# bcgsc/ntJoin

Hardware: AMD Instinct MI355X
Metric: Gbp/s minimizer-sketch+graph-build (k=32,w=1000) (higher is better)
Workload: dtype u64

## Files before the change

ntjoin_amd/csrc/graph.hip:

```cpp
#include <algorithm>
#include <cstdlib>
#include <cstring>
#include <system_error>
#include <thread>

#include "join_verdict.h"
#include "graph_rank.h"
#include "mxg_internal.h"
#include "scan_kernels.h"

namespace mxg {

static constexpr uint64_t HT_EMPTY = 0xFFFFFFFFFFFFFFFFull;
static constexpr uint32_t NONE32 = 0xFFFFFFFFu;

struct Slot {
    unsigned long long key;
    uint32_t nseen, ndup;
};

__device__ __forceinline__ uint32_t ht_slot(Slot *tab, uint32_t mask, uint32_t cap, uint64_t key)
{
    if (key == HT_EMPTY) return cap;
    uint32_t s = (uint32_t)((key * 0x9E3779B97F4A7C15ull) >> 32) & mask;
// ... 65 lines not shown

__global__ __launch_bounds__(256) void k_flags(const AsmSet p, const Slot *__restrict__ tab, uint32_t *cnt, uint32_t *sup)
{
    const uint32_t a = asm_of_block(p, blockIdx.x);
    const uint32_t i = (blockIdx.x - p.bstart[a]) * 256u + threadIdx.x;
    bool sh = false;
    if (i < asm_n(p, a)) {
        const uint32_t bit = 1u << a, full = p.full;
        const Slot sl = tab[p.slot[a][i]];
        const uint32_t seen = ~sl.nseen & full, d = ~sl.ndup & full;
        const bool uniq = !(d & bit);
        const bool inall = seen == full;
        sh = inall && d == 0;
        p.flags[a][i] = (uint8_t)((uniq ? MXG_MX_UNIQUE : 0) | (sh ? MXG_MX_SHARED : 0) | (inall ? MXG_MX_INALL : 0));
    }
    const uint32_t c = (uint32_t)__syncthreads_count(sh ? 1 : 0);
    if (threadIdx.x == 0) count_publish(cnt + p.bstart[a], sup + sup_start(p, a), blockIdx.x - p.bstart[a], c);
}


__device__ __forceinline__ uint32_t pj_part(uint64_t key, uint32_t pmask)
{
    return (uint32_t)((key * 0x9E3779B97F4A7C15ull) >> 44) & pmask;
}

constexpr uint32_t PJ_REC_DUP = 0x80000000u;
__device__ __forceinline__ uint32_t pj_run_role(uint32_t i, uint32_t n, uint64_t key, bool live)
{
    const uint32_t lane = threadIdx.x & 63u;
    const uint64_t prev = __shfl_up(key, 1), next = __shfl_down(key, 1);
    const bool fol = live && lane > 0 && prev == key;
    const bool lead = live && !fol && lane < 63 && i + 1 < n && next == key;
    return (fol ? 1u : 0u) | (lead ? 2u : 0u);
}

constexpr uint32_t PJ_BT = 1024;
__global__ __launch_bounds__(PJ_BT) void k_pj_bucket(const AsmSet p, uint32_t nb, uint32_t pmask, uint32_t *M, uint4 *recs,
                                                   uint32_t *sup, uint32_t n_sup)
{
    extern __shared__ uint32_t pj_lds[];
    uint32_t *hist = pj_lds, *start = pj_lds + pmask + 1;
    __shared__ uint32_t sh[256];
    if (blockIdx.x == 0)
        for (uint32_t i = threadIdx.x; i < n_sup; i += PJ_BT) sup[i] = 0;
    constexpr uint32_t U = PJ_IPB / PJ_BT;
    constexpr uint32_t BPU = PJ_BT / 256;
    const uint32_t j = blockIdx.x, sub = threadIdx.x >> 8, t256 = threadIdx.x & 255u;
    const uint32_t blk0 = j * (PJ_IPB / 256), a0 = asm_of_block(p, blk0), a1 = asm_of_block(p, min(blk0 + PJ_IPB / 256, nb) - 1u);
    const bool one = a0 == a1;
    const uint64_t *hp0 = p.hash[a0];
    uint32_t *sp0 = p.slot[a0];
    const uint32_t n0 = asm_n(p, a0), ib0 = (blk0 - p.bstart[a0]) * 256u;
    uint64_t key[U];
    uint32_t live = 0, dupm = 0;
#pragma unroll
    for (uint32_t u = 0; u < U; ++u) {
        const uint32_t blk = blk0 + u * BPU + sub;
        key[u] = 0;
        if (blk >= nb) continue;
        const uint64_t *hp = hp0;
        uint32_t *sp = sp0;
        uint32_t i = ib0 + (u * BPU + sub) * 256u + t256, n = n0;
        if (!one) {
            const uint32_t a = asm_of_block(p, blk);
            hp = p.hash[a];
            sp = p.slot[a];
            i = (blk - p.bstart[a]) * 256u + t256;
            n = asm_n(p, a);
        }
        const bool lv = i < n;
        if (lv) {
            key[u] = hp[i];
            sp[i] = PJ_VERDICT_PREFILL;
        }
        const uint32_t role = pj_run_role(i, n, key[u], lv);
        const uint64_t fb = __ballot(role & 1u);
        if ((threadIdx.x & 63u) == 0) p.fol[(size_t)blk * 4u + ((threadIdx.x >> 6) & 3u)] = fb;
        if (lv && !(role & 1u)) live |= 1u << u;
        if (role & 2u) dupm |= 1u << u;
    }
    for (uint32_t b = threadIdx.x; b <= pmask; b += PJ_BT) hist[b] = 0;
    __syncthreads();
#pragma unroll
    for (uint32_t u = 0; u < U; ++u)
        if ((live >> u) & 1u) atomicAdd(&hist[pj_part(key[u], pmask)], 1u);
    __syncthreads();
    const uint32_t P = pmask + 1, per = P >= PJ_BT ? P / PJ_BT : 1u, b0 = threadIdx.x * per;
    uint32_t c = 0;
    if (b0 < P)
        for (uint32_t u = 0; u < per; ++u) c += hist[b0 + u];
    uint32_t run = block_exclusive<PJ_BT / 64>(c, sh);
    uint32_t *row = M + (size_t)j * (P + 1);
    if (b0 < P)
        for (uint32_t u = 0; u < per; ++u) {
            const uint32_t cb = hist[b0 + u];
            start[b0 + u] = run;
            row[b0 + u] = run;
            hist[b0 + u] = 0;
            run += cb;
        }
    if (threadIdx.x == 0) row[P] = sh[255];
    __syncthreads();
#pragma unroll
    for (uint32_t u = 0; u < U; ++u) {
        if (!((live >> u) & 1u)) continue;
        const uint32_t blk = blk0 + u * BPU + sub;
        uint32_t a = a0, i = ib0 + (u * BPU + sub) * 256u + t256;
        if (!one) {
            a = asm_of_block(p, blk);
            i = (blk - p.bstart[a]) * 256u + t256;
        }
        const uint32_t b = pj_part(key[u], pmask);
        const uint32_t pos = j * PJ_IPB + start[b] + atomicAdd(&hist[b], 1u);
        recs[pos] = make_uint4((uint32_t)key[u], (uint32_t)(key[u] >> 32), i, a | (((dupm >> u) & 1u) ? PJ_REC_DUP : 0u));
    }
}

__device__ __forceinline__ uint32_t pj_slot_from(unsigned long long *keys, uint64_t key, uint32_t s)
{
    if (key == HT_EMPTY) return PJ_T;
    for (uint32_t step = 0; step < PJ_T; ++step) {
        const unsigned long long cur = keys[s];
        if (cur == key) return s;
        if (cur == HT_EMPTY) {
            const unsigned long long old = atomicCAS(&keys[s], (unsigned long long)HT_EMPTY, (unsigned long long)key);
            if (old == HT_EMPTY || old == key) return s;
        }
        s = (s + 1u) & (PJ_T - 1u);
    }
    return PJ_T + 1u;
}
__device__ __forceinline__ uint32_t pj_slot(unsigned long long *keys, uint64_t key)
{
    return pj_slot_from(keys, key, (uint32_t)((key * 0x9E3779B97F4A7C15ull) >> 32) & (PJ_T - 1u));
}

struct PjRec3 {
    uint32_t x, y, z;
};
template <bool R12>
__device__ __forceinline__ uint4 pj_rec_load(const uint4 *recs, size_t r)
{
    if (!R12) return recs[r];
    const PjRec3 v = reinterpret_cast<const PjRec3 *>(recs)[r];
    return make_uint4(v.x, v.y, v.z, 0u);
}
template <bool R12>
__device__ __forceinline__ void pj_rec_store(uint4 *recs, size_t r, const uint4 v)
{
    if (!R12) recs[r] = v;
    else reinterpret_cast<PjRec3 *>(recs)[r] = PjRec3{v.x, v.y, v.z};
}

struct PjSub {
    uint32_t n_sub, s, off, cap;
};
struct PjSubCaps {
    uint32_t n_sub;
    uint32_t cap[MXG_MAX_ASSEMBLIES];
};
template <bool NARROW>
__global__ __launch_bounds__(256) void k_pj_join(uint4 *recs, const uint32_t *__restrict__ M, uint32_t P, uint32_t n_rows,
                                                 uint64_t *host_fail, uint32_t force_fail, const uint32_t *__restrict__ cursor,
                                                 uint32_t cap1, uint32_t rows2, const AsmSet p, const PjSubCaps caps, uint32_t prefill0)
{
    const uint32_t full = p.full;
    __shared__ unsigned long long keys[PJ_T + 1];
    __shared__ uint32_t seen[PJ_T + 1], dup[NARROW ? 1 : PJ_T + 1];
    __shared__ uint32_t item0[PJ_T + 1];
    __shared__ uint32_t seg_off[257], seg_rec[256], sh[256];
    __shared__ uint32_t failed;
    uint32_t b = blockIdx.x, rec_off = 0;
    if (cursor) {
        const uint32_t c = blockIdx.x / P;
        b = blockIdx.x % P;
        n_rows = caps.n_sub > 1 ? rows2 : (min(cursor[c * PJ1_CS], cap1) + PJ_IPB - 1) / PJ_IPB;
        M += (size_t)c * rows2 * (P + 1);
        rec_off = c * cap1;
        if (threadIdx.x == 0)
            for (uint32_t s = 0; s < caps.n_sub; ++s)
                if (cursor[(c * caps.n_sub + s) * PJ1_CS] > caps.cap[s]) *host_fail = 1;
    }
    for (uint32_t s = threadIdx.x; s <= PJ_T; s += 256) {
        keys[s] = HT_EMPTY;
        seen[s] = 0;
        if (!NARROW) dup[s] = 0;
    }
    if (threadIdx.x == 0) failed = force_fail;
    constexpr uint32_t QC = 4;
    uint32_t rc[QC], sc[QC], ac[QC], ic[QC];
    const bool single = n_rows <= 256;
    for (uint32_t pass = 0; pass < 2; ++pass) {
        const bool bad = pass == 1 && failed != 0;
        if (bad && threadIdx.x == 0) *host_fail = 1;
        for (uint32_t j0 = 0; j0 < n_rows; j0 += 256) {
            if (pass == 0 || !single) {
                const uint32_t j = j0 + threadIdx.x;
                uint32_t lo = 0, len = 0;
                if (j < n_rows) {
                    const uint32_t *row = M + (size_t)j * (P + 1);
                    lo = row[b];
                    len = row[b + 1] - lo;
                }
                const uint32_t off = block_exclusive_256(len, sh);
                seg_off[threadIdx.x] = off;
                seg_rec[threadIdx.x] = rec_off + j * PJ_IPB + lo;
                __syncthreads();
            }
            const uint32_t total = sh[255];
            auto locate = [&](uint32_t q) {
                uint32_t l = 0, h = 256;
                while (h - l > 1) {
                    const uint32_t m = (l + h) >> 1;
                    if (seg_off[m] <= q) l = m; else h = m;
                }
                return seg_rec[l] + (q - seg_off[l]);
            };
            uint32_t last_a = 0, last_i = 0;
            auto insert_rec = [&](const uint4 rec) {
                last_a = rec.w & ~PJ_REC_DUP;
                last_i = rec.z;
                const uint32_t s = pj_slot(keys, ((uint64_t)rec.y << 32) | rec.x);
                if (pass == 0) {
                    const uint32_t bit = 1u << last_a;
                    if (s > PJ_T) failed = 1;
                    else {
                        const uint32_t cur = seen[s], dcur = NARROW ? cur >> 16 : dup[s];
                        if (!((cur & bit) && (dcur & bit))) {
                            if (rec.w & PJ_REC_DUP) {
                                if (NARROW) atomicOr(&seen[s], bit | (bit << 16));
                                else {
                                    atomicOr(&seen[s], bit);
                                    atomicOr(&dup[s], bit);
                                }
                            } else if (atomicOr(&seen[s], bit) & bit) {
                                if (NARROW) atomicOr(&seen[s], bit << 16); else atomicOr(&dup[s], bit);
                            }
                            if (last_a == 0) item0[s] = rec.z;
                        }
                    }
                }
                return s;
            };
            auto insert = [&](uint32_t r) { return insert_rec(recs[r]); };
            auto finish = [&](uint32_t i, uint32_t s, uint32_t a) {
                uint32_t fl = 0;
                if (!bad) {
                    const uint32_t sn = seen[s] & full, d = (NARROW ? seen[s] >> 16 : dup[s]) & full;
                    const bool inall = sn == full;
                    fl = (!(d & (1u << a)) ? MXG_MX_UNIQUE : 0u) | ((inall && d == 0) ? MXG_MX_SHARED : 0u) | (inall ? MXG_MX_INALL : 0u);
                }
                const uint32_t word = ((fl & MXG_MX_SHARED) ? item0[s] << 3 : 0u) | fl;
                if (word != pj_verdict_prefill(prefill0, a, i)) p.slot[a][i] = word;
            };
#pragma unroll
            for (uint32_t it = 0; it < QC; ++it) {
                const uint32_t q = threadIdx.x + it * 256u;
                if (q >= total) break;
                if (pass == 0) {
                    rc[it] = locate(q);
                    sc[it] = insert(rc[it]);
                    ac[it] = last_a;
                    ic[it] = last_i;
                } else if (single) {
                    finish(ic[it], sc[it], ac[it]);
                } else {
                    const uint32_t r = locate(q);
                    const uint32_t s = insert(r);
                    finish(last_i, s, last_a);
                }
            }
            constexpr uint32_t TU = 8;
            for (uint32_t q0 = threadIdx.x + QC * 256u; q0 < total; q0 += 256u * TU) {
                uint4 rv[TU];
#pragma unroll
                for (uint32_t u = 0; u < TU; ++u) {
                    const uint32_t q = q0 + u * 256u;
                    rv[u] = q < total ? recs[locate(q)] : make_uint4(0u, 0u, 0u, 0u);
                }
#pragma unroll
                for (uint32_t u = 0; u < TU; ++u) {
                    if (q0 + u * 256u >= total) break;
                    const uint32_t s = insert_rec(rv[u]);
                    if (pass == 1) finish(last_i, s, last_a);
                }
            }
            __syncthreads();
        }
    }
}


template <bool NARROW, bool R12>
__global__ __launch_bounds__(256) void k_pj_join_pipe(uint4 *recs, const uint32_t *__restrict__ M, uint32_t P, uint32_t n_parts,
                                                      uint64_t *host_fail, uint32_t force_fail, const uint32_t *__restrict__ cursor,
                                                      uint32_t cap1, uint32_t rows2, const AsmSet p, const PjSubCaps caps, uint32_t prefill0)
{
    const uint32_t full = p.full;
    const uint32_t lgP = R12 ? 31u - (uint32_t)__clz(P) : 0u, tag_mask = R12 ? pj12_tag_mask(lgP) : 0u;
    auto rec_a = [&](const uint4 rec) { return R12 ? pj12_unpack_tag(rec.y, lgP) & (PJ12_TAG_DUP - 1u) : rec.w & ~PJ_REC_DUP; };
    auto rec_dup = [&](const uint4 rec) { return R12 ? (pj12_unpack_tag(rec.y, lgP) & PJ12_TAG_DUP) != 0 : (rec.w & PJ_REC_DUP) != 0; };
    auto rec_slot = [&](unsigned long long *tab, const uint4 rec) {
        if (R12) return pj_slot_from(tab, ((uint64_t)(rec.y & ~tag_mask) << 32) | rec.x, rec.y & (PJ_T - 1u));
        return pj_slot(tab, ((uint64_t)rec.y << 32) | rec.x);
    };
    __shared__ unsigned long long keys[PJ_T + 1];
    __shared__ uint32_t seen[PJ_T + 1], dup[NARROW ? 1 : PJ_T + 1];
    __shared__ uint32_t item0[PJ_T + 1];
    __shared__ uint32_t seg_off[2][257], seg_rec[2][256], sh[256];
    __shared__ uint32_t failed;
    constexpr uint32_t QC = 4;
    __shared__ uint8_t seg_of[QC * 256];
    uint4 rn[QC];
    uint32_t tot_n = 0;
    uint32_t lo_nn = 0, len_nn = 0;
    auto bounds = [&](uint32_t part, uint32_t &lo, uint32_t &len) {
        lo = len = 0;
        if (part < n_parts && threadIdx.x < rows2) {
            const uint32_t c = part / P, b = part % P;
            const uint32_t *row = M + ((size_t)c * rows2 + threadIdx.x) * (P + 1);
            lo = row[b];
            len = row[b + 1];
        }
    };
    auto lay_out = [&](uint32_t part, uint32_t buf, uint32_t lo, uint32_t end) {
        const uint32_t c = part < n_parts ? part / P : 0u;
        const uint32_t len = end - lo;
        const uint32_t off = block_exclusive_256(len, sh);
        seg_off[buf][threadIdx.x] = off;
        seg_rec[buf][threadIdx.x] = c * cap1 + threadIdx.x * PJ_IPB + lo;
        for (uint32_t q = off, e = min(off + len, QC * 256u); q < e; ++q) seg_of[q] = (uint8_t)threadIdx.x;
        const uint32_t total = sh[255];
        __syncthreads();
#pragma unroll
        for (uint32_t it = 0; it < QC; ++it) {
            const uint32_t q = threadIdx.x + it * 256u;
            rn[it] = make_uint4(0u, 0u, 0u, 0u);
            if (q < total) {
                const uint32_t l = seg_of[q];
                rn[it] = pj_rec_load<R12>(recs, seg_rec[buf][l] + (q - seg_off[buf][l]));
            }
        }
        return total;
    };
    const uint32_t first = blockIdx.x, stride = gridDim.x;
    {
        uint32_t lo, end;
        bounds(first, lo, end);
        bounds(first + stride, lo_nn, len_nn);
        tot_n = lay_out(first, 0u, lo, end);
    }
    uint32_t k = 0;
    for (uint32_t part = first; part < n_parts; part += stride, ++k) {
        uint4 rc[QC];
#pragma unroll
        for (uint32_t it = 0; it < QC; ++it) rc[it] = rn[it];
        const uint32_t total = tot_n, buf = k & 1u;
        {
            const uint32_t lo = lo_nn, end = len_nn;
            bounds(part + 2u * stride, lo_nn, len_nn);
            tot_n = lay_out(part + stride, buf ^ 1u, lo, end);
        }
        for (uint32_t s = threadIdx.x; s <= PJ_T; s += 256) {
            keys[s] = HT_EMPTY;
            seen[s] = 0;
            if (!NARROW) dup[s] = 0;
        }
        if (threadIdx.x == 0) {
            failed = force_fail;
            const uint32_t c = part / P;
            if (part % P == 0)
                for (uint32_t s = 0; s < caps.n_sub; ++s)
                    if (cursor[(c * caps.n_sub + s) * PJ1_CS] > caps.cap[s]) *host_fail = 1;
        }
        __syncthreads();
        auto locate = [&](uint32_t q) {
            uint32_t l = 0, h = 256;
            while (h - l > 1) {
                const uint32_t m = (l + h) >> 1;
                if (seg_off[buf][m] <= q) l = m; else h = m;
            }
            return seg_rec[buf][l] + (q - seg_off[buf][l]);
        };
        auto insert_rec = [&](const uint4 rec, bool record) {
            const uint32_t a = rec_a(rec);
            const uint32_t s = rec_slot(keys, rec);
            if (record) {
                const uint32_t bit = 1u << a;
                if (s > PJ_T) failed = 1;
                else {
                    const uint32_t cur = seen[s], dcur = NARROW ? cur >> 16 : dup[s];
                    if (!((cur & bit) && (dcur & bit))) {
                        if (rec_dup(rec)) {
                            if (NARROW) atomicOr(&seen[s], bit | (bit << 16));
                            else {
                                atomicOr(&seen[s], bit);
                                atomicOr(&dup[s], bit);
                            }
                        } else if (atomicOr(&seen[s], bit) & bit) {
                            if (NARROW) atomicOr(&seen[s], bit << 16); else atomicOr(&dup[s], bit);
                        }
                        if (a == 0) item0[s] = rec.z;
                    }
                }
            }
            return s;
        };
        uint32_t sc[QC];
#pragma unroll
        for (uint32_t it = 0; it < QC; ++it)
            if (threadIdx.x + it * 256u < total) sc[it] = insert_rec(rc[it], true);
        constexpr uint32_t TU = 8;
        for (uint32_t q0 = threadIdx.x + QC * 256u; q0 < total; q0 += 256u * TU) {
            uint4 rv[TU];
#pragma unroll
            for (uint32_t u = 0; u < TU; ++u) {
                const uint32_t q = q0 + u * 256u;
                rv[u] = q < total ? pj_rec_load<R12>(recs, locate(q)) : make_uint4(0u, 0u, 0u, 0u);
            }
#pragma unroll
            for (uint32_t u = 0; u < TU; ++u)
                if (q0 + u * 256u < total) insert_rec(rv[u], true);
        }
        __syncthreads();
        const bool bad = failed != 0;
        if (bad && threadIdx.x == 0) *host_fail = 1;
        auto finish = [&](const uint4 rec, uint32_t s) {
            const uint32_t a = rec_a(rec);
            uint32_t fl = 0;
            if (!bad) {
                const uint32_t sn = seen[s] & full, d = (NARROW ? seen[s] >> 16 : dup[s]) & full;
                const bool inall = sn == full;
                fl = (!(d & (1u << a)) ? MXG_MX_UNIQUE : 0u) | ((inall && d == 0) ? MXG_MX_SHARED : 0u) | (inall ? MXG_MX_INALL : 0u);
            }
            const uint32_t word = ((fl & MXG_MX_SHARED) ? item0[s] << 3 : 0u) | fl;
            if (word != pj_verdict_prefill(prefill0, a, rec.z)) p.slot[a][rec.z] = word;
        };
#pragma unroll
        for (uint32_t it = 0; it < QC; ++it)
            if (threadIdx.x + it * 256u < total) finish(rc[it], bad ? 0u : sc[it]);
        for (uint32_t q0 = threadIdx.x + QC * 256u; q0 < total; q0 += 256u * TU) {
            uint4 rv[TU];
#pragma unroll
            for (uint32_t u = 0; u < TU; ++u) {
                const uint32_t q = q0 + u * 256u;
                rv[u] = q < total ? pj_rec_load<R12>(recs, locate(q)) : make_uint4(0u, 0u, 0u, 0u);
            }
#pragma unroll
            for (uint32_t u = 0; u < TU; ++u)
                if (q0 + u * 256u < total) finish(rv[u], bad ? 0u : insert_rec(rv[u], false));
        }
        __syncthreads();
    }
}

__device__ __forceinline__ uint32_t pj1_part(uint64_t key, uint32_t p1mask) { return (uint32_t)((key * 0x9E3779B97F4A7C15ull) >> 52) & p1mask; }

template <bool R12, uint32_t G>
__global__ __launch_bounds__(PJ_BT) void k_pj1_scatter(const AsmSet p, uint32_t blk_lo, uint32_t blk_hi, uint32_t p1mask, uint32_t cap1,
                                                     uint32_t *cursor, uint4 *recs1, uint32_t *sup, uint32_t n_sup, const PjSub subr,
                                                     uint32_t prefill0)
{
    auto part1 = [&](uint64_t k) { return R12 ? (uint32_t)(k >> 52) & p1mask : pj1_part(k, p1mask); };
    extern __shared__ uint32_t pj_lds[];
    uint32_t *hist = pj_lds, *start = pj_lds + p1mask + 1;
    if (blockIdx.x == 0)
        for (uint32_t i = threadIdx.x; i < n_sup; i += PJ_BT) sup[i] = 0;
    constexpr uint32_t U = PJ_IPB / PJ_BT, BPU = PJ_BT / 256, NU = U * G;
    const uint32_t j = blockIdx.x;
    const uint32_t blk0 = blk_lo + j * (G * (PJ_IPB / 256));
    auto blk_of = [&](uint32_t u, uint32_t t) { return blk0 + (u / U) * (PJ_IPB / 256) + (u % U) * BPU + (t >> 8); };
    auto thread_again = [] {
        uint32_t t = threadIdx.x;
        asm volatile("" : "+v"(t));
        return t;
    };
    const bool own = R12 || subr.n_sub > 1;
    const uint32_t bs_own = p.bstart[subr.s], n_own = own ? asm_n(p, subr.s) : 0u;
    uint64_t key[NU];
    uint32_t ia[R12 ? 1 : NU], ii[R12 ? 1 : NU], live = 0, dupm = 0;
    const uint32_t t_a = thread_again();
#pragma unroll
    for (uint32_t u = 0; u < NU; ++u) {
        const uint32_t blk = blk_of(u, t_a), in = blk < blk_hi, t256 = t_a & 255u;
        const uint32_t a = own ? subr.s : asm_of_block(p, min(blk, blk_hi - 1u));
        const uint32_t i = (blk - (own ? bs_own : p.bstart[a])) * 256u + t256, n = own ? n_own : asm_n(p, a);
        const bool lv = in && i < n;
        key[u] = p.hash[a][lv ? i : 0u];
        if (lv) p.slot[a][i] = pj_verdict_prefill(prefill0, a, i);
    }
    const uint32_t t_b = thread_again();
#pragma unroll
    for (uint32_t u = 0; u < NU; ++u) {
        const uint32_t blk = blk_of(u, t_b), in = blk < blk_hi, t256 = t_b & 255u;
        const uint32_t a = own ? subr.s : asm_of_block(p, min(blk, blk_hi - 1u));
        const uint32_t i = (blk - (own ? bs_own : p.bstart[a])) * 256u + t256, n = own ? n_own : asm_n(p, a);
        const bool lv = in && i < n;
        const uint32_t role = pj_run_role(i, n, key[u], lv);
        const uint64_t fb = __ballot(role & 1u);
        if (in && (threadIdx.x & 63u) == 0) p.fol[(size_t)blk * 4u + ((threadIdx.x >> 6) & 3u)] = fb;
        if (R12) key[u] *= PJ_MUL;
        const bool rec = lv && !(role & 1u);
        if (!R12) {
            ia[u] = rec ? a | ((role & 2u) ? PJ_REC_DUP : 0u) : 0u;
            ii[u] = rec ? i : 0u;
        }
        dupm |= rec && (role & 2u) ? 1u << u : 0u;
        live |= rec ? 1u << u : 0u;
    }
    asm volatile("" : "+v"(live), "+v"(dupm));
#pragma unroll
    for (uint32_t u = 0; u < NU; ++u) asm volatile("" : "+v"(key[u]));
    for (uint32_t b = threadIdx.x; b <= p1mask; b += PJ_BT) hist[b] = 0;
    __syncthreads();
#pragma unroll
    for (uint32_t u = 0; u < NU; ++u)
        if ((live >> u) & 1u) atomicAdd(&hist[part1(key[u])], 1u);
    __syncthreads();
    for (uint32_t b = threadIdx.x; b <= p1mask; b += PJ_BT) {
        const uint32_t c = hist[b];
        start[b] = c ? atomicAdd(&cursor[(b * subr.n_sub + subr.s) * PJ1_CS], c) : 0u;
        hist[b] = 0;
    }
    __syncthreads();
    const uint32_t t_c = thread_again();
#pragma unroll
    for (uint32_t u = 0; u < NU; ++u) {
        if (!((live >> u) & 1u)) continue;
        const uint32_t b = part1(key[u]);
        const uint32_t pos = start[b] + atomicAdd(&hist[b], 1u);
        const uint32_t i = R12 ? (blk_of(u, t_c) - bs_own) * 256u + (t_c & 255u) : ii[u], aw = R12 ? subr.s : ia[u];
        if (pos < subr.cap)
            pj_rec_store<R12>(recs1, (size_t)b * cap1 + subr.off + pos,
                              make_uint4((uint32_t)key[u], (uint32_t)(key[u] >> 32), R12 && ((dupm >> u) & 1u) ? i | PJ12_ITEM_DUP : i, aw));
        else p.slot[aw & ~PJ_REC_DUP][i] = 0;
    }
}

template <bool R12>
__global__ __launch_bounds__(PJ_BT) void k_pj2_bucket(const AsmSet p, const uint4 *__restrict__ recs1, const uint32_t *__restrict__ cursor,
                                                    uint32_t cap1, uint32_t rows2, uint32_t pmask, uint32_t *M, uint4 *recs2,
                                                    uint32_t skew_lim, const PjSub subr)
{
    extern __shared__ uint32_t pj_lds[];
    uint32_t *hist = pj_lds, *start = pj_lds + pmask + 1;
    __shared__ uint32_t sh[256];
    const uint32_t j = blockIdx.x, c = blockIdx.y;
    const uint32_t lgP = R12 ? 31u - (uint32_t)__clz(pmask + 1u) : 0u;
    auto part2 = [&](const uint4 r) { return R12 ? (r.y >> PJ12_FINE_SHIFT) & pmask : pj_part(((uint64_t)r.y << 32) | r.x, pmask); };
    const uint32_t n_all = cursor[(c * subr.n_sub + subr.s) * PJ1_CS], n_c = min(n_all, subr.cap);
    const uint32_t row_j = subr.off / PJ_IPB + j;
    if (j * PJ_IPB >= n_c) {
        uint32_t *row = M + ((size_t)c * rows2 + row_j) * (pmask + 2);
        for (uint32_t b = threadIdx.x; b <= pmask + 1; b += PJ_BT) row[b] = 0;
        return;
    }
    constexpr uint32_t U = PJ_IPB / PJ_BT;
    const size_t base = (size_t)c * cap1 + subr.off + (size_t)j * PJ_IPB;
    uint4 rec[U];
    uint32_t live = 0;
#pragma unroll
    for (uint32_t u = 0; u < U; ++u) {
        const uint32_t q = u * PJ_BT + threadIdx.x;
        rec[u] = make_uint4(0u, 0u, 0u, 0u);
        if (j * PJ_IPB + q < n_c) {
            rec[u] = pj_rec_load<R12>(recs1, base + q);
            if (R12) {
                rec[u].w = subr.s | ((rec[u].z & PJ12_ITEM_DUP) ? PJ_REC_DUP : 0u);
                rec[u].z &= ~PJ12_ITEM_DUP;
            }
            live |= 1u << u;
        }
    }
    if (n_all > skew_lim) {
        __shared__ unsigned long long skey[PJ_IPB];
        __shared__ uint32_t sitem[PJ_IPB];
        __shared__ uint8_t sasm[PJ_IPB];
        __shared__ uint32_t stab[PJ_IPB];
        __shared__ uint32_t sdup[PJ_IPB / 32];
        for (uint32_t q = threadIdx.x; q < PJ_IPB; q += PJ_BT) stab[q] = 0xFFFFFFFFu;
        for (uint32_t q = threadIdx.x; q < PJ_IPB / 32; q += PJ_BT) sdup[q] = 0;
#pragma unroll
        for (uint32_t u = 0; u < U; ++u) {
            const uint32_t q = u * PJ_BT + threadIdx.x;
            skey[q] = ((unsigned long long)rec[u].y << 32) | rec[u].x;
            sitem[q] = rec[u].z;
            sasm[q] = (uint8_t)(rec[u].w & 0xFFu);
        }
        __syncthreads();
#pragma unroll
        for (uint32_t u = 0; u < U; ++u) {
            if (!((live >> u) & 1u)) continue;
            const uint32_t q = u * PJ_BT + threadIdx.x;
            const unsigned long long key = skey[q];
            const uint32_t a = rec[u].w & 0xFFu;
            uint32_t hsl = (uint32_t)(((key + a) * 0x9E3779B97F4A7C15ull) >> 40) & (2u * PJ_IPB - 1u);
            uint32_t rep = q;
            for (;;) {
                const uint32_t sft = (hsl & 1u) * 16u;
                const uint32_t word = stab[hsl >> 1], cur = (word >> sft) & 0xFFFFu;
                if (cur == 0xFFFFu) {
                    const uint32_t want = (word & ~(0xFFFFu << sft)) | (q << sft);
                    if (atomicCAS(&stab[hsl >> 1], word, want) == word) break;
                    continue;
                }
                if (skey[cur] == key && sasm[cur] == a) {
                    rep = cur;
                    break;
                }
                hsl = (hsl + 1u) & (2u * PJ_IPB - 1u);
            }
            if (rep != q) {
                atomicOr(&sdup[rep >> 5], 1u << (rep & 31u));
                p.slot[a][rec[u].z] = (sitem[rep] << 3) | PJ_VERDICT_REF;
                live &= ~(1u << u);
            }
        }
        __syncthreads();
#pragma unroll
        for (uint32_t u = 0; u < U; ++u) {
            const uint32_t q = u * PJ_BT + threadIdx.x;
            if ((sdup[q >> 5] >> (q & 31u)) & 1u) rec[u].w |= PJ_REC_DUP;
        }
    }
    for (uint32_t b = threadIdx.x; b <= pmask; b += PJ_BT) hist[b] = 0;
    __syncthreads();
#pragma unroll
    for (uint32_t u = 0; u < U; ++u)
        if ((live >> u) & 1u) atomicAdd(&hist[part2(rec[u])], 1u);
    __syncthreads();
    const uint32_t P = pmask + 1, per = P >= PJ_BT ? P / PJ_BT : 1u, b0 = threadIdx.x * per;
    uint32_t cn = 0;
    if (b0 < P)
        for (uint32_t u = 0; u < per; ++u) cn += hist[b0 + u];
    uint32_t run = block_exclusive<PJ_BT / 64>(cn, sh);
    uint32_t *row = M + ((size_t)c * rows2 + row_j) * (P + 1);
    if (b0 < P)
        for (uint32_t u = 0; u < per; ++u) {
            const uint32_t cb = hist[b0 + u];
            start[b0 + u] = run;
            row[b0 + u] = run;
            hist[b0 + u] = 0;
            run += cb;
        }
    if (threadIdx.x == 0) row[P] = sh[255];
    __syncthreads();
#pragma unroll
    for (uint32_t u = 0; u < U; ++u) {
        if (!((live >> u) & 1u)) continue;
        const uint32_t b = part2(rec[u]);
        const uint32_t pos = (uint32_t)base + start[b] + atomicAdd(&hist[b], 1u);
        if (R12) rec[u].y = pj12_pack(rec[u].y, lgP, pj12_tag(rec[u].w & ~PJ_REC_DUP, (rec[u].w & PJ_REC_DUP) != 0));
        pj_rec_store<R12>(recs2, pos, rec[u]);
    }
}

template <uint32_t U>
struct TailScan {
    uint32_t tot[U][4];
    uint32_t before[U];
};
template <uint32_t U>
__device__ __forceinline__ void tail_ballot(TailScan<U> &ts, uint32_t u, bool f, uint64_t &bm)
{
    bm = __ballot(f);
    if ((threadIdx.x & 63u) == 0) ts.tot[u][threadIdx.x >> 6] = (uint32_t)__popcll(bm);
}
template <uint32_t U>
__device__ __forceinline__ uint32_t tail_rank(const TailScan<U> &ts, uint32_t u, uint64_t bm)
{
    const uint32_t lane = threadIdx.x & 63u, wv = threadIdx.x >> 6;
    uint32_t r = (uint32_t)__popcll(bm & ((1ull << lane) - 1ull));
#pragma unroll
    for (uint32_t q = 0; q < 3; ++q) r += q < wv ? ts.tot[u][q] : 0u;
    return r;
}
template <uint32_t U>
__device__ __forceinline__ uint32_t tail_total(const TailScan<U> &ts, uint32_t u)
{
    return ts.tot[u][0] + ts.tot[u][1] + ts.tot[u][2] + ts.tot[u][3];
}

struct TailAsm {
    uint32_t a, n, b0;
};
__device__ __forceinline__ TailAsm tail_asm(const AsmSet &p, uint32_t a)
{
    return TailAsm{a, asm_n(p, a), p.bstart[a]};
}
template <uint32_t U>
__device__ __forceinline__ bool tail_asms(const AsmSet &p, uint32_t blk0, uint32_t nb, TailAsm (&t)[U])
{
    const uint32_t a_first = asm_of_block(p, blk0), a_last = U > 1 ? asm_of_block(p, min(blk0 + U, nb) - 1u) : a_first;
    t[0] = tail_asm(p, a_first);
#pragma unroll
    for (uint32_t u = 1; u < U; ++u) t[u] = t[0];
    if (a_first != a_last) {
#pragma unroll
        for (uint32_t u = 1; u < U; ++u)
            if (blk0 + u < nb) t[u] = tail_asm(p, asm_of_block(p, blk0 + u));
    }
    return a_first == a_last;
}

template <uint32_t U>
__global__ __launch_bounds__(256) void k_flags_pj(const AsmSet p, uint32_t nb, uint32_t *cnt, uint32_t *sup, uint64_t *mask0)
{
    __shared__ TailScan<U> ts;
    const uint32_t blk0 = blockIdx.x * U, lane = threadIdx.x & 63u, wv = threadIdx.x >> 6;
    TailAsm t[U];
    tail_asms<U>(p, blk0, nb, t);
    uint64_t fb[U];
    uint32_t v[U], ia[U], ii[U];
    bool in[U];
#pragma unroll
    for (uint32_t u = 0; u < U; ++u) {
        const bool there = blk0 + u < nb;
        const uint32_t blk = there ? blk0 + u : blk0;
        ia[u] = t[u].a;
        ii[u] = (blk - t[u].b0) * 256u + threadIdx.x;
        in[u] = there && ii[u] < t[u].n;
        fb[u] = p.fol[(size_t)blk * 4u + wv];
        v[u] = p.slot[t[u].a][in[u] ? ii[u] : 0u];
    }
#pragma unroll
    for (uint32_t u = 0; u < U; ++u) {
        if (blk0 + u >= nb) fb[u] = 0;
        if (!in[u]) v[u] = 0;
    }
    bool other[U];
#pragma unroll
    for (uint32_t u = 0; u < U; ++u) {
        const bool isf = (fb[u] >> lane) & 1ull;
        if (isf) v[u] = 0u;
        other[u] = isf;
        if ((v[u] & 7u) == PJ_VERDICT_REF) {
            v[u] = p.slot[ia[u]][v[u] >> 3];
            other[u] = true;
        }
    }
#pragma unroll
    for (uint32_t u = 0; u < U; ++u) {
        const bool isf = (fb[u] >> lane) & 1ull;
        const uint32_t lead = 63u - (uint32_t)__clzll(~fb[u] & ((2ull << lane) - 1ull));
        const uint32_t vl = __shfl(v[u], lead);
        uint32_t w = isf ? vl : v[u];
        if (other[u]) w &= MXG_MX_INALL;
        const bool sh = in[u] && (w & MXG_MX_SHARED) != 0;
        if (in[u]) p.flags[ia[u]][ii[u]] = (uint8_t)(w & 7u);
        uint64_t bm;
        tail_ballot(ts, u, sh, bm);
        if (blk0 + u < nb && ia[u] == 0 && lane == 0) mask0[(size_t)(blk0 + u - p.bstart[0]) * 4u + wv] = bm;
    }
    __syncthreads();
    if (wv < U && lane == 0 && blk0 + wv < nb) {
        const uint32_t blk = blk0 + wv, a = asm_of_block(p, blk);
        count_publish(cnt + p.bstart[a], sup + sup_start(p, a), blk - p.bstart[a], tail_total(ts, wv));
    }
}

struct VertexParams {
    const uint8_t *flags;
    const uint32_t *cnt, *sup;
    uint64_t *n_shared;
    const uint32_t *slot;
    const uint64_t *hash;
    const uint32_t *pos, *rec;
// ... 680 lines not shown
                       pl.as_all, pl.recs1, pl.cursor, pl.cap1, pl.rows2, pl.P - 1, pl.M, pl.recs2,
                       knob_u64(h, "MXG_PJ_SKEW", 0) ? 0u : skew_lim, sub);
}

static int ev_pair(mxg_handle *h, hipEvent_t *a, hipEvent_t *b)
{
    while (h->ev_pool.size() < h->ev_used + 2) {
        hipEvent_t e;
        MXG_HIP(h, hipEventCreate(&e));
        h->ev_pool.push_back(e);
    }
    *a = h->ev_pool[h->ev_used];
    *b = h->ev_pool[h->ev_used + 1];
    h->ev_used += 2;
    h->ev_spans.push_back(TimedSpan{*a, *b, 0, false, 5});
    return MXG_OK;
}

int graph_plan_early(mxg_handle *h, const GraphBounds &gb, bool *early)
{
    *early = false;
    h->pj_early_done = 0;
    if (knob_u64(h, "MXG_PJ_EARLY", 1) == 0) return MXG_OK;
    MXG_HIP(h, hipSetDevice(h->device));
    if (!h->pj_plan) h->pj_plan = new JoinPlan;
    JoinPlan &pl = *h->pj_plan;
    const std::string err_before = h->err;
    if (plan_join(h, GRAPH_FULL, &gb, h->pj_learnt.overflowed, true, pl) != MXG_OK || !(pl.pj && pl.two_level && pl.split && pl.nb)) {
        pl = JoinPlan();
        h->err = err_before;
        return MXG_OK;
    }
    MXG_HIP(h, hipMemsetAsync(pl.fsup, 0, pl.clear_words * 4, h->stream));
    if (!h->ev_plan) MXG_HIP(h, hipEventCreateWithFlags(&h->ev_plan, hipEventDisableTiming));
    MXG_HIP(h, hipEventRecord(h->ev_plan, h->stream));
    *early = true;
    return MXG_OK;
}

int graph_partition_early(mxg_handle *h, uint32_t a, hipStream_t st)
{
    const JoinPlan *pl = h->pj_plan;
    if (!pl || !pl->split || a != h->pj_early_done || a >= pl->A) return MXG_OK;
    if (h->asms[a]->d_hash.as<uint64_t>() != pl->as_all.hash[a] || h->asms[a]->d_slot.as<uint32_t>() != pl->as_all.slot[a]) return MXG_OK;
    if (st != h->stream) MXG_HIP(h, hipStreamWaitEvent(st, h->ev_plan, 0));
    const bool fine = (h->cfg.flags & MXG_FLAG_TIMING_FINE) != 0;
    hipEvent_t e0 = nullptr, e1 = nullptr;
    if (fine) {
        const int rc = ev_pair(h, &e0, &e1);
        if (rc != MXG_OK) return rc;
        MXG_HIP(h, hipEventRecord(e0, st));
    }
    launch_partition(h, *pl, a, a + 1, st, 0u);
    MXG_HIP(h, hipGetLastError());
    if (fine) MXG_HIP(h, hipEventRecord(e1, st));
    ++h->pj_early_done;
    return MXG_OK;
}

void graph_drop_plan(mxg_handle *h)
{
    delete h->pj_plan;
    h->pj_plan = nullptr;
}

static int take_or_make_plan(mxg_handle *h, const GraphCall &c, bool global_table, JoinPlan &own, const JoinPlan **plan)
{
    const JoinPlan *ep = h->pj_plan;
    bool early = ep && ep->split && h->pj_early_done != 0 && h->pj_early_done == ep->A && c.gb && c.mode == GRAPH_FULL && !global_table &&
                 ep->A == h->asms.size();
    for (uint32_t a = 0; early && a < ep->A; ++a) early = c.gb->n_bound[a] == ep->n_of[a] && c.gb->n_ptr[a] == ep->as_all.n_ptr[a];
    h->pj_early_done = 0;
    *plan = early ? ep : &own;
    if (early) return MXG_OK;
    const int rc = plan_join(h, c.mode, c.gb, global_table, false, own);
    if (rc != MXG_OK && c.mode != GRAPH_DG_EDGES && c.mode != GRAPH_DG_EDGES_APPLIED)
        for (Assembly *a : h->asms) a->flags_valid = a->flags_on_host = false;
    return rc;
}

#define TAIL_LAUNCH(kernel, U, grid, stream, ...)                                                      \
    do {                                                                                               \
        if ((U) == 4) hipLaunchKernelGGL(kernel<4>, grid, dim3(256), 0, stream, __VA_ARGS__);          \
        else if ((U) == 2) hipLaunchKernelGGL(kernel<2>, grid, dim3(256), 0, stream, __VA_ARGS__);     \
        else hipLaunchKernelGGL(kernel<1>, grid, dim3(256), 0, stream, __VA_ARGS__);                   \
    } while (0)

#define TAIL_LAUNCH2(kernel, U, X, grid, stream, ...)                                                  \
    do {                                                                                               \
        if ((U) == 4) hipLaunchKernelGGL((kernel<4, X>), grid, dim3(256), 0, stream, __VA_ARGS__);     \
        else if ((U) == 2) hipLaunchKernelGGL((kernel<2, X>), grid, dim3(256), 0, stream, __VA_ARGS__); \
        else hipLaunchKernelGGL((kernel<1, X>), grid, dim3(256), 0, stream, __VA_ARGS__);              \
    } while (0)

struct GraphStage {
    mxg_handle *const h;
    const GraphCall &c;
    const JoinPlan &pl;
    const bool early;
    const bool resume;
    const bool fine, timing;
    Graph &g;
    uint64_t *ctl = nullptr, *hctl = nullptr;
    uint64_t *pj_fail = nullptr;

    GraphStage(mxg_handle *h_, const GraphCall &c_, const JoinPlan &pl_, bool early_)
        : h(h_), c(c_), pl(pl_), early(early_), resume(c_.mode == GRAPH_DG_EDGES || c_.mode == GRAPH_DG_EDGES_APPLIED),
          fine((h_->cfg.flags & MXG_FLAG_TIMING_FINE) != 0 && c_.mode == GRAPH_FULL), timing((h_->cfg.flags & MXG_FLAG_TIMING) != 0 || fine),
          g(h_->graph)
    {
    }
    bool joins() const { return pl.nb && !resume; }
    size_t anv() const { return (size_t)pl.A * pl.nvs; }

    int begin()
    {
        for (uint32_t ai = 0; ai < pl.A; ++ai) {
            Assembly *a = h->asms[ai];
            if (!resume) a->flags_on_host = false;
            a->flags_valid = true;
        }
        if (!resume) g = Graph();
        g.n_asm = pl.A;
        if (fine && !h->ev_g[0]) {
            MXG_HIP(h, hipEventCreate(&h->ev_g[0]));
            MXG_HIP(h, hipEventCreate(&h->ev_g[1]));
        }
        if (timing) MXG_HIP(h, hipEventRecord(h->ev0, h->stream));
        if (!resume)
            h->stat_graph_join = (pl.pj ? (pl.two_level ? MXG_JOIN_LDS_TWO_LEVEL : MXG_JOIN_LDS) : MXG_JOIN_GLOBAL) | (early ? MXG_JOIN_EARLY : 0);
        if (!resume && knob_u64(h, "MXG_DEBUG_JOIN", 0)) {
            uint32_t t1 = 0;
            for (uint32_t a = 0; pl.pj && pl.two_level && a < (pl.split ? pl.A : 1u); ++a)
                t1 = std::max(t1, pj1_launch_tiles(pl, pl.split ? a : 0u, pl.split ? a + 1 : pl.A));
            fprintf(stderr, "[mxg] join pj=%d two_level=%d split=%d early=%d record_bytes=%d prefill0=%u P1=%u rows2=%u tiles1=%u rank=%d\n",
                    (int)pl.pj, (int)pl.two_level, (int)pl.split, (int)early, pl.rec12 ? 12 : 16, pl.prefill0, pl.P1, pl.rows2, t1, (int)pl.graph_rank);
        }
        if (!pl.pj && !resume) MXG_HIP(h, hipMemsetAsync(h->g_keys.p, 0xFF, ((size_t)pl.cap + 1) * sizeof(Slot), h->stream));
        ctl = h->g_ctl.as<uint64_t>();
        if (!h->pinned_gctl) MXG_HIP(h, hipHostMalloc((void **)&h->pinned_gctl, CTL_WORDS * 8));
        hctl = h->pinned_gctl;
        memset(hctl, 0, CTL_WORDS * 8);
        pj_fail = pl.dg_pj ? dg_pj_fail_word(h) : hctl + CTL_PJ_FAIL;
        return MXG_OK;
    }

    void launch_join(uint4 *recs, uint32_t *M, uint32_t n_parts, uint32_t n_rows, const uint32_t *cursor)
    {
        const bool narrow = pl.A <= 16;
        const uint32_t cap1 = cursor ? pl.cap1 : 0u, rows2 = cursor ? pl.rows2 : 0u;
        const uint64_t pipe_blocks = cursor ? knob_u64(h, "MXG_PJ_PIPE", 1024) : 0;
        const uint32_t prefill0 = cursor ? pl.prefill0 : 0u;
        if (pipe_blocks && rows2 <= 256) {
            auto kernel = pl.rec12 ? (narrow ? k_pj_join_pipe<true, true> : k_pj_join_pipe<false, true>)
                                   : (narrow ? k_pj_join_pipe<true, false> : k_pj_join_pipe<false, false>);
            hipLaunchKernelGGL(kernel, dim3((uint32_t)std::min<uint64_t>(pipe_blocks, n_parts)), dim3(256), 0, h->stream, recs, M, pl.P, n_parts,
                               pj_fail, pl.pj_force_fail, cursor, cap1, rows2, pl.as_all, pl.sc, prefill0);
        } else
            hipLaunchKernelGGL(narrow ? k_pj_join<true> : k_pj_join<false>, dim3(n_parts), dim3(256), 0, h->stream, recs, M, pl.P, n_rows,
                               pj_fail, pl.pj_force_fail, cursor, cap1, rows2, pl.as_all, pl.sc, prefill0);
    }
    void flags_pj()
    {
        TAIL_LAUNCH(k_flags_pj, pl.u_flags, dim3(graph_tail_grid(pl.nb, pl.u_flags)), h->stream, pl.as_all, pl.nb, pl.cnt, pl.fsup, pl.pj_mask0);
    }
    int join_two_level()
    {
        if (!early && pl.split) {
            MXG_HIP(h, hipMemsetAsync(pl.fsup, 0, pl.clear_words * 4, h->stream));
            for (uint32_t a = 0; a < pl.A; ++a) launch_partition(h, pl, a, a + 1, h->stream, 0u);
        } else if (!early) {
            MXG_HIP(h, hipMemsetAsync(pl.cursor, 0, (size_t)pl.P1 * PJ1_CS * 4, h->stream));
            launch_partition(h, pl, 0, pl.A, h->stream, pl.n_fsup + pl.n_esup);
        }
        launch_join(pl.recs2, pl.M, pl.P1 * pl.P, 0u, pl.cursor);
        flags_pj();
        return MXG_OK;
    }
    int join_one_level()
    {
        const uint32_t n_rows = (pl.nb + PJ_IPB / 256 - 1) / (PJ_IPB / 256);
        MXG_HIP(h, h->g_part.ensure((size_t)n_rows * (pl.P + 1) * 4));
        MXG_HIP(h, h->g_keys.ensure((size_t)n_rows * PJ_IPB * sizeof(uint4)));
        uint32_t *M = h->g_part.as<uint32_t>();
        uint4 *recs = h->g_keys.as<uint4>();
        hipLaunchKernelGGL(k_pj_bucket, dim3(n_rows), dim3(PJ_BT), (size_t)pl.P * 8, h->stream, pl.as_all, pl.nb, pl.P - 1, M, recs, pl.fsup,
                           pl.n_fsup + pl.n_esup);
        launch_join(recs, M, pl.P, n_rows, nullptr);
        flags_pj();
        return MXG_OK;
    }
    int join_global()
    {
        hipLaunchKernelGGL(k_insert, dim3(pl.nb), dim3(256), 0, h->stream, pl.as_all, h->g_keys.as<Slot>(), pl.mask, pl.cap, pl.fsup,
                           pl.n_fsup + pl.n_esup);
        hipLaunchKernelGGL(k_flags, dim3(pl.nb), dim3(256), 0, h->stream, pl.as_all, h->g_keys.as<Slot>(), pl.cnt, pl.fsup);
        return MXG_OK;
    }
    int mark(hipEvent_t ev)
    {
        MXG_HIP(h, hipGetLastError());
        if (fine) MXG_HIP(h, hipEventRecord(ev, h->stream));
        return MXG_OK;
    }

    int vertex_arrays()
    {
        MXG_HIP(h, h->g_vhash.ensure(pl.nvs * 8));
        MXG_HIP(h, h->g_vpos.ensure(anv() * 4));
        MXG_HIP(h, h->g_vrec.ensure(anv() * 4));
        MXG_HIP(h, h->g_fv.ensure(anv() * 4));
        MXG_HIP(h, h->g_frec.ensure(anv() * 4));
        MXG_HIP(h, h->g_nxt.ensure(2 * anv() * 4));
        if (c.mode == GRAPH_DG_EDGES) MXG_HIP(h, hipMemsetAsync(h->g_nxt.p, 0xFF, 2 * anv() * 4, h->stream));
        return MXG_OK;
    }
    int item_vids(uint32_t a, uint32_t **ivid)
    {
        *ivid = nullptr;
        if (c.mode != GRAPH_DG_VERTICES) return MXG_OK;
        MXG_HIP(h, h->asms[a]->d_ivid.ensure((size_t)pl.n_of[a] * 4 + 16));
        *ivid = h->asms[a]->d_ivid.as<uint32_t>();
        return MXG_OK;
    }
    int fill(VertexPjParams &vp)
    {
        vp.as = pl.as_all;
        for (uint32_t a = 0; a < MXG_MAX_ASSEMBLIES; ++a) {
            vp.pos[a] = a < pl.A ? h->asms[a]->d_pos.as<uint32_t>() : nullptr;
            vp.rec[a] = a < pl.A ? h->asms[a]->d_rec.as<uint32_t>() : nullptr;
            vp.ivid[a] = nullptr;
            int rc;
            if (a < pl.A && (rc = item_vids(a, &vp.ivid[a])) != MXG_OK) return rc;
        }
        vp.cnt = pl.cnt;
        vp.sup = pl.fsup;
        vp.n_shared = ctl + CTL_SHARED;
        vp.mask0 = pl.pj_mask0;
        vp.bpref0 = pl.pj_bpref0;
        vp.vhash = h->g_vhash.as<uint64_t>();
        vp.vpos = h->g_vpos.as<uint32_t>();
        vp.vrec = h->g_vrec.as<uint32_t>();
        vp.fv = h->g_fv.as<uint32_t>();
        vp.frec = h->g_frec.as<uint32_t>();
        vp.rank = pl.graph_rank ? h->g_nxt.as<uint32_t>() : nullptr;
        vp.nvs = (uint32_t)pl.nvs;
        return MXG_OK;
    }
    int vertices_pj()
    {
        VertexPjParams vp;
        const int rc = fill(vp);
        if (rc != MXG_OK) return rc;
        hipLaunchKernelGGL(k_block_prefix, dim3((uint32_t)((pl.nb0 + 255) / 256)), dim3(256), 0, h->stream, pl.cnt + pl.as_all.bstart[0],
                           pl.fsup + sup_start(pl.as_all, 0), (uint32_t)pl.nb0, pl.pj_bpref0);
        TAIL_LAUNCH(k_vertices_pj, pl.u_vertices, dim3(graph_tail_grid(pl.nb, pl.u_vertices)), h->stream, vp, pl.nb);
        return MXG_OK;
    }
    int fill(VertexParams &vp, uint32_t a)
    {
        Assembly *as = h->asms[a];
        const size_t row = (size_t)a * pl.nvs;
        vp.flags = as->d_flags.as<uint8_t>();
        vp.cnt = pl.cnt + pl.as_all.bstart[a];
        vp.sup = pl.fsup + sup_start(pl.as_all, a);
        vp.n_shared = ctl + CTL_SHARED + a;
        vp.slot = as->d_slot.as<uint32_t>();
        vp.hash = as->d_hash.as<uint64_t>();
        vp.pos = as->d_pos.as<uint32_t>();
        vp.rec = as->d_rec.as<uint32_t>();
        vp.n = (uint32_t)pl.n_of[a];
        vp.n_ptr = c.gb ? c.gb->n_ptr[a] : nullptr;
        vp.first = a == 0;
        vp.vid = h->g_vid.as<uint32_t>();
        vp.vhash = h->g_vhash.as<uint64_t>();
        vp.vpos = h->g_vpos.as<uint32_t>() + row;
        vp.vrec = h->g_vrec.as<uint32_t>() + row;
        vp.fv = h->g_fv.as<uint32_t>() + row;
        vp.frec = h->g_frec.as<uint32_t>() + row;
        return item_vids(a, &vp.ivid);
    }
    int vertices_global()
    {
        for (uint32_t a = 0; a < pl.A; ++a) {
            VertexParams vp;
            const int rc = fill(vp, a);
            if (rc != MXG_OK) return rc;
            if (vp.ivid) MXG_HIP(h, hipMemsetAsync(vp.ivid, 0xFF, (size_t)vp.n * 4, h->stream));
            hipLaunchKernelGGL(k_vertices, dim3((vp.n + 255) / 256), dim3(256), 0, h->stream, vp);
        }
        return MXG_OK;
    }
    int hand_back_vertices()
    {
        g.nv_stride = pl.nvs;
        if (!c.d_n_vertices) return MXG_OK;
        if (pl.nvs > 0) MXG_HIP(h, hipMemcpyAsync(c.d_n_vertices, ctl + CTL_SHARED, 8, hipMemcpyDeviceToDevice, h->stream));
        else MXG_HIP(h, hipMemsetAsync(c.d_n_vertices, 0, 8, h->stream));
        return MXG_OK;
    }

    void adjacency_own()
    {
        TAIL_LAUNCH(k_adjacency, pl.u_edges, dim3(graph_tail_grid((pl.nvs + 255) / 256, pl.u_edges), pl.A), h->stream, h->g_fv.as<uint32_t>(),
                    h->g_frec.as<uint32_t>(), ctl + CTL_SHARED, h->g_nxt.as<uint2>(), (uint32_t)pl.nvs);
    }
    void adjacency_of_owner()
    {
// ... 182 lines not shown
```

ntjoin_amd/csrc/join_verdict.h:

```cpp
#pragma once
#include <cstdint>

#include "ntjoin_mx.h"

#if defined(__HIPCC__)
#define PJV_HD __host__ __device__ inline
#else
#define PJV_HD inline
#endif

namespace mxg {

constexpr uint32_t PJ_VERDICT_PREFILL = MXG_MX_UNIQUE;
constexpr uint32_t PJ_VERDICT_REF = 2u;

PJV_HD bool pj_verdict_is_prefill(uint32_t word) { return word == PJ_VERDICT_PREFILL; }

enum PjPrefillRule : uint32_t { PJ_PREFILL_UNIQUE = 0, PJ_PREFILL_OWN0 = 1 };
constexpr uint32_t PJ_VERDICT_SHARED = MXG_MX_UNIQUE | MXG_MX_SHARED | MXG_MX_INALL;

PJV_HD uint32_t pj_verdict_prefill(uint32_t rule, uint32_t a, uint32_t i)
{
    return rule == PJ_PREFILL_OWN0 && a == 0 ? (i << 3) | PJ_VERDICT_SHARED : PJ_VERDICT_PREFILL;
}

}
```

Measured before the change: 2821.

## Make join-kernel record loads branchless and defer verdict stores across pipeline iterations

Measured after the change: 2838, median of 6. No clear change (+0.6%).

```diff
diff --git a/ntjoin_amd/csrc/graph.hip b/ntjoin_amd/csrc/graph.hip
--- a/ntjoin_amd/csrc/graph.hip
+++ b/ntjoin_amd/csrc/graph.hip
@@ -241,6 +241,8 @@
     else reinterpret_cast<PjRec3 *>(recs)[r] = PjRec3{v.x, v.y, v.z};
 }
 
+__device__ __forceinline__ void pj_rec_arrived(const uint4 &r) { asm volatile("" ::"v"(r.x), "v"(r.y), "v"(r.z), "v"(r.w)); }
+
 struct PjSub {
     uint32_t n_sub, s, off, cap;
 };
@@ -248,6 +250,27 @@
     uint32_t n_sub;
     uint32_t cap[MXG_MAX_ASSEMBLIES];
 };
+struct PjSlotTab {
+    uint32_t *of[MXG_MAX_ASSEMBLIES];
+};
+static_assert(sizeof(PjSlotTab) == PJ_SLOT_TAB_BYTES, "one address per assembly");
+__device__ __forceinline__ void pj_slot_tab_fill(PjSlotTab &tab, const AsmSet &p)
+{
+    if (threadIdx.x < p.n_asm) tab.of[threadIdx.x] = p.slot[threadIdx.x];
+}
+__device__ __forceinline__ void pj_slot_store(const PjSlotTab &tab, uint32_t a, uint32_t i, uint32_t word)
+{
+    typedef uint32_t __attribute__((address_space(1))) *global_u32;
+    ((global_u32)tab.of[a])[i] = word;
+}
+__device__ __forceinline__ uint32_t pj_seg_of(const uint32_t *seg_off, uint32_t q)
+{
+    uint32_t l = 0;
+#pragma unroll
+    for (uint32_t step = 128; step != 0; step >>= 1) l += seg_off[l + step] <= q ? step : 0u;
+    return l;
+}
+
 template <bool NARROW>
 __global__ __launch_bounds__(256) void k_pj_join(uint4 *recs, const uint32_t *__restrict__ M, uint32_t P, uint32_t n_rows,
                                                  uint64_t *host_fail, uint32_t force_fail, const uint32_t *__restrict__ cursor,
@@ -259,6 +282,8 @@
     __shared__ uint32_t item0[PJ_T + 1];
     __shared__ uint32_t seg_off[257], seg_rec[256], sh[256];
     __shared__ uint32_t failed;
+    __shared__ PjSlotTab slot_tab;
+    pj_slot_tab_fill(slot_tab, p);
     uint32_t b = blockIdx.x, rec_off = 0;
     if (cursor) {
         const uint32_t c = blockIdx.x / P;
@@ -298,11 +323,7 @@
             }
             const uint32_t total = sh[255];
             auto locate = [&](uint32_t q) {
-                uint32_t l = 0, h = 256;
-                while (h - l > 1) {
-                    const uint32_t m = (l + h) >> 1;
-                    if (seg_off[m] <= q) l = m; else h = m;
-                }
+                const uint32_t l = pj_seg_of(seg_off, q);
                 return seg_rec[l] + (q - seg_off[l]);
             };
             uint32_t last_a = 0, last_i = 0;
@@ -340,7 +361,7 @@
                     fl = (!(d & (1u << a)) ? MXG_MX_UNIQUE : 0u) | ((inall && d == 0) ? MXG_MX_SHARED : 0u) | (inall ? MXG_MX_INALL : 0u);
                 }
                 const uint32_t word = ((fl & MXG_MX_SHARED) ? item0[s] << 3 : 0u) | fl;
-                if (word != pj_verdict_prefill(prefill0, a, i)) p.slot[a][i] = word;
+                if (word != pj_verdict_prefill(prefill0, a, i)) pj_slot_store(slot_tab, a, i, word);
             };
 #pragma unroll
             for (uint32_t it = 0; it < QC; ++it) {
@@ -365,7 +386,7 @@
 #pragma unroll
                 for (uint32_t u = 0; u < TU; ++u) {
                     const uint32_t q = q0 + u * 256u;
-                    rv[u] = q < total ? recs[locate(q)] : make_uint4(0u, 0u, 0u, 0u);
+                    rv[u] = recs[locate(q < total ? q : 0u)];
                 }
 #pragma unroll
                 for (uint32_t u = 0; u < TU; ++u) {
@@ -373,6 +394,8 @@
                     const uint32_t s = insert_rec(rv[u]);
                     if (pass == 1) finish(last_i, s, last_a);
                 }
+#pragma unroll
+                for (uint32_t u = 0; u < TU; ++u) pj_rec_arrived(rv[u]);
             }
             __syncthreads();
         }
@@ -380,7 +403,7 @@
 }
 
 
-template <bool NARROW, bool R12>
+template <bool NARROW, bool R12, bool DEFER>
 __global__ __launch_bounds__(256) void k_pj_join_pipe(uint4 *recs, const uint32_t *__restrict__ M, uint32_t P, uint32_t n_parts,
                                                       uint64_t *host_fail, uint32_t force_fail, const uint32_t *__restrict__ cursor,
                                                       uint32_t cap1, uint32_t rows2, const AsmSet p, const PjSubCaps caps, uint32_t prefill0)
@@ -400,7 +423,9 @@
     __shared__ uint32_t failed;
     constexpr uint32_t QC = 4;
     __shared__ uint8_t seg_of[QC * 256];
-    uint4 rn[QC];
+    __shared__ PjSlotTab slot_tab;
+    pj_slot_tab_fill(slot_tab, p);
+    uint4 rn[QC] = {};
     uint32_t tot_n = 0;
     uint32_t lo_nn = 0, len_nn = 0;
     auto bounds = [&](uint32_t part, uint32_t &lo, uint32_t &len) {
@@ -422,15 +447,25 @@
         const uint32_t total = sh[255];
         __syncthreads();
 #pragma unroll
-        for (uint32_t it = 0; it < QC; ++it) {
-            const uint32_t q = threadIdx.x + it * 256u;
-            rn[it] = make_uint4(0u, 0u, 0u, 0u);
-            if (q < total) {
-                const uint32_t l = seg_of[q];
-                rn[it] = pj_rec_load<R12>(recs, seg_rec[buf][l] + (q - seg_off[buf][l]));
+        for (uint32_t it = 0; it < QC; ++it) rn[it] = make_uint4(0u, 0u, 0u, 0u);
+        if (total != 0) {
+#pragma unroll
+            for (uint32_t it = 0; it < QC; ++it) {
+                const uint32_t q = threadIdx.x + it * 256u, qq = q < total ? q : 0u;
+                const uint32_t l = seg_of[qq];
+                rn[it] = pj_rec_load<R12>(recs, seg_rec[buf][l] + (qq - seg_off[buf][l]));
             }
         }
         return total;
+    };
+    typedef uint32_t __attribute__((address_space(1))) *global_u32;
+    global_u32 pend_at[QC];
+    uint32_t pend_word[QC], pend = 0;
+    auto store_pending = [&] {
+#pragma unroll
+        for (uint32_t it = 0; it < QC; ++it)
+            if ((pend >> it) & 1u) *pend_at[it] = pend_word[it];
+        pend = 0;
     };
     const uint32_t first = blockIdx.x, stride = gridDim.x;
     {
@@ -444,6 +479,7 @@
         uint4 rc[QC];
 #pragma unroll
         for (uint32_t it = 0; it < QC; ++it) rc[it] = rn[it];
+        if (DEFER) store_pending();
         const uint32_t total = tot_n, buf = k & 1u;
         {
             const uint32_t lo = lo_nn, end = len_nn;
@@ -464,11 +500,7 @@
         }
         __syncthreads();
         auto locate = [&](uint32_t q) {
-            uint32_t l = 0, h = 256;
-            while (h - l > 1) {
-                const uint32_t m = (l + h) >> 1;
-                if (seg_off[buf][m] <= q) l = m; else h = m;
-            }
+            const uint32_t l = pj_seg_of(seg_off[buf], q);
             return seg_rec[buf][l] + (q - seg_off[buf][l]);
         };
         auto insert_rec = [&](const uint4 rec, bool record) {
@@ -505,16 +537,18 @@
 #pragma unroll
             for (uint32_t u = 0; u < TU; ++u) {
                 const uint32_t q = q0 + u * 256u;
-                rv[u] = q < total ? pj_rec_load<R12>(recs, locate(q)) : make_uint4(0u, 0u, 0u, 0u);
+                rv[u] = pj_rec_load<R12>(recs, locate(q < total ? q : 0u));
             }
 #pragma unroll
             for (uint32_t u = 0; u < TU; ++u)
                 if (q0 + u * 256u < total) insert_rec(rv[u], true);
+#pragma unroll
+            for (uint32_t u = 0; u < TU; ++u) pj_rec_arrived(rv[u]);
         }
         __syncthreads();
         const bool bad = failed != 0;
         if (bad && threadIdx.x == 0) *host_fail = 1;
-        auto finish = [&](const uint4 rec, uint32_t s) {
+        auto finish = [&](const uint4 rec, uint32_t s, uint32_t keep) {
             const uint32_t a = rec_a(rec);
             uint32_t fl = 0;
             if (!bad) {
@@ -523,24 +557,33 @@
                 fl = (!(d & (1u << a)) ? MXG_MX_UNIQUE : 0u) | ((inall && d == 0) ? MXG_MX_SHARED : 0u) | (inall ? MXG_MX_INALL : 0u);
             }
             const uint32_t word = ((fl & MXG_MX_SHARED) ? item0[s] << 3 : 0u) | fl;
-            if (word != pj_verdict_prefill(prefill0, a, rec.z)) p.slot[a][rec.z] = word;
+            if (word != pj_verdict_prefill(prefill0, a, rec.z)) {
+                if (DEFER && keep < QC) {
+                    pend_at[keep] = (global_u32)slot_tab.of[a] + rec.z;
+                    pend_word[keep] = word;
+                    pend |= 1u << keep;
+                } else pj_slot_store(slot_tab, a, rec.z, word);
+            }
         };
 #pragma unroll
         for (uint32_t it = 0; it < QC; ++it)
-            if (threadIdx.x + it * 256u < total) finish(rc[it], bad ? 0u : sc[it]);
+            if (threadIdx.x + it * 256u < total) finish(rc[it], bad ? 0u : sc[it], it);
         for (uint32_t q0 = threadIdx.x + QC * 256u; q0 < total; q0 += 256u * TU) {
             uint4 rv[TU];
 #pragma unroll
             for (uint32_t u = 0; u < TU; ++u) {
                 const uint32_t q = q0 + u * 256u;
-                rv[u] = q < total ? pj_rec_load<R12>(recs, locate(q)) : make_uint4(0u, 0u, 0u, 0u);
+                rv[u] = pj_rec_load<R12>(recs, locate(q < total ? q : 0u));
             }
 #pragma unroll
             for (uint32_t u = 0; u < TU; ++u)
-                if (q0 + u * 256u < total) finish(rv[u], bad ? 0u : insert_rec(rv[u], false));
+                if (q0 + u * 256u < total) finish(rv[u], bad ? 0u : insert_rec(rv[u], false), QC);
+#pragma unroll
+            for (uint32_t u = 0; u < TU; ++u) pj_rec_arrived(rv[u]);
         }
         __syncthreads();
     }
+    if (DEFER) store_pending();
 }
 
 __device__ __forceinline__ uint32_t pj1_part(uint64_t key, uint32_t p1mask) { return (uint32_t)((key * 0x9E3779B97F4A7C15ull) >> 52) & p1mask; }
@@ -646,19 +689,22 @@
     }
     constexpr uint32_t U = PJ_IPB / PJ_BT;
     const size_t base = (size_t)c * cap1 + subr.off + (size_t)j * PJ_IPB;
+    const uint32_t n_here = min(n_c - j * PJ_IPB, PJ_IPB);
     uint4 rec[U];
     uint32_t live = 0;
 #pragma unroll
     for (uint32_t u = 0; u < U; ++u) {
         const uint32_t q = u * PJ_BT + threadIdx.x;
-        rec[u] = make_uint4(0u, 0u, 0u, 0u);
-        if (j * PJ_IPB + q < n_c) {
-            rec[u] = pj_rec_load<R12>(recs1, base + q);
-            if (R12) {
-                rec[u].w = subr.s | ((rec[u].z & PJ12_ITEM_DUP) ? PJ_REC_DUP : 0u);
-                rec[u].z &= ~PJ12_ITEM_DUP;
-            }
-            live |= 1u << u;
+        const bool lv = q < n_here;
+        rec[u] = pj_rec_load<R12>(recs1, base + (lv ? q : 0u));
+        live |= lv ? 1u << u : 0u;
+    }
+#pragma unroll
+    for (uint32_t u = 0; u < U; ++u) {
+        if (!((live >> u) & 1u)) rec[u] = make_uint4(0u, 0u, 0u, 0u);
+        else if (R12) {
+            rec[u].w = subr.s | ((rec[u].z & PJ12_ITEM_DUP) ? PJ_REC_DUP : 0u);
+            rec[u].z &= ~PJ12_ITEM_DUP;
         }
     }
     if (n_all > skew_lim) {
@@ -667,6 +713,8 @@
         __shared__ uint8_t sasm[PJ_IPB];
         __shared__ uint32_t stab[PJ_IPB];
         __shared__ uint32_t sdup[PJ_IPB / 32];
+        __shared__ PjSlotTab slot_tab;
+        pj_slot_tab_fill(slot_tab, p);
         for (uint32_t q = threadIdx.x; q < PJ_IPB; q += PJ_BT) stab[q] = 0xFFFFFFFFu;
         for (uint32_t q = threadIdx.x; q < PJ_IPB / 32; q += PJ_BT) sdup[q] = 0;
 #pragma unroll
@@ -701,7 +749,7 @@
             }
             if (rep != q) {
                 atomicOr(&sdup[rep >> 5], 1u << (rep & 31u));
-                p.slot[a][rec[u].z] = (sitem[rep] << 3) | PJ_VERDICT_REF;
+                pj_slot_store(slot_tab, a, rec[u].z, (sitem[rep] << 3) | PJ_VERDICT_REF);
                 live &= ~(1u << u);
             }
         }
@@ -1688,8 +1736,11 @@
         const uint64_t pipe_blocks = cursor ? knob_u64(h, "MXG_PJ_PIPE", 1024) : 0;
         const uint32_t prefill0 = cursor ? pl.prefill0 : 0u;
         if (pipe_blocks && rows2 <= 256) {
-            auto kernel = pl.rec12 ? (narrow ? k_pj_join_pipe<true, true> : k_pj_join_pipe<false, true>)
-                                   : (narrow ? k_pj_join_pipe<true, false> : k_pj_join_pipe<false, false>);
+            const bool defer = knob_u64(h, "MXG_PJ_DEFER", 1) != 0;
+            auto kernel = defer ? (pl.rec12 ? (narrow ? k_pj_join_pipe<true, true, true> : k_pj_join_pipe<false, true, true>)
+                                            : (narrow ? k_pj_join_pipe<true, false, true> : k_pj_join_pipe<false, false, true>))
+                                : (pl.rec12 ? (narrow ? k_pj_join_pipe<true, true, false> : k_pj_join_pipe<false, true, false>)
+                                            : (narrow ? k_pj_join_pipe<true, false, false> : k_pj_join_pipe<false, false, false>));
             hipLaunchKernelGGL(kernel, dim3((uint32_t)std::min<uint64_t>(pipe_blocks, n_parts)), dim3(256), 0, h->stream, recs, M, pl.P, n_parts,
                                pj_fail, pl.pj_force_fail, cursor, cap1, rows2, pl.as_all, pl.sc, prefill0);
         } else
diff --git a/ntjoin_amd/csrc/join_verdict.h b/ntjoin_amd/csrc/join_verdict.h
--- a/ntjoin_amd/csrc/join_verdict.h
+++ b/ntjoin_amd/csrc/join_verdict.h
@@ -19,6 +19,8 @@
 enum PjPrefillRule : uint32_t { PJ_PREFILL_UNIQUE = 0, PJ_PREFILL_OWN0 = 1 };
 constexpr uint32_t PJ_VERDICT_SHARED = MXG_MX_UNIQUE | MXG_MX_SHARED | MXG_MX_INALL;
 
+constexpr uint32_t PJ_SLOT_TAB_BYTES = MXG_MAX_ASSEMBLIES * 8;
+
 PJV_HD uint32_t pj_verdict_prefill(uint32_t rule, uint32_t a, uint32_t i)
 {
     return rule == PJ_PREFILL_OWN0 && a == 0 ? (i << 3) | PJ_VERDICT_SHARED : PJ_VERDICT_PREFILL;
```
